# ZeayW/Multimodal-fusion-based-Pre-routing-Timing-Prediction-

Measured on AMD Instinct MI355X. Metric: train-step samples/sec, higher is better.
Workload: dtype bf16; 1 GPU; config B: 8 designs/step/GPU, 65536-node netlist, 64 levels, 256x256 tile, 1350 endpoints/design, UNet(max), bf16 operands / fp32 accumulate on the MFMA-bound contractions; U-Net activations and their gradients stored bf16, netlist tensors, statistics, parameters and gradients fp32; nodes=65536, levels=64, tile=256, endpoints_per_design=1350, cone_pruning=False, parallelism=dp1 (designs sharded, one all-reduce of the flat gradient per step), launch=one HIP graph replay per step (Adam inside)

## Files before the change

include/mmft.h:

```cpp
#ifndef MMFT_H_
#define MMFT_H_

#ifdef __cplusplus
extern "C" {
#endif

#define MMFT_OK 0
#define MMFT_ERR_BAD_ARG (-1)
#define MMFT_ERR_UNSUPPORTED (-2)
#define MMFT_ERR_LAUNCH (-3)

#define MMFT_EPI_STORE 0
#define MMFT_EPI_ACCUM 1
#define MMFT_EPI_ADD_ACT 2
#define MMFT_ACT_NONE 0
#define MMFT_ACT_RELU 1
#define MMFT_ACT_LEAKY 2
#define MMFT_POOL_MAX 0
#define MMFT_POOL_AVG 1

int mmft_version(void);
const char* mmft_last_error(void);
#define MMFT_MATH_F32 0
#define MMFT_MATH_BF16 1
// ... 232 lines not shown
int mmft_u16_pack_weights(const void* descs, int n, long long max_frag_lanes, long long* counters, int ncounters, long long inc,
                          int device, void* stream);
int mmft_u16_conv_tiles(int N, int H, int W, int* per_image);
int mmft_u16_conv3x3(const void* x, int rgb_f32, const void* wpk, void* y, float* stats, int N, int H, int W, int Ci, int Co,
                     int device, void* stream);
long long mmft_u16_conv3x3_wgrad_workspace_bytes(int N, int H, int W, int Ci, int Co);
int mmft_u16_conv3x3_wgrad_slabs(int N, int H, int W, int Ci, int Co);
int mmft_u16_conv3x3_wgrad(const void* x, int rgb_f32, const void* dy, float* dw, int accumulate, int N, int H, int W, int Ci,
                           int Co, float* workspace, long long workspace_bytes, int device, void* stream);
int mmft_u16_bn_finalize(const float* stats, int tiles_per_image, int N, int C, long long pixels_per_image, float eps,
                         const float* gamma, const float* beta, float* bnp, int device, void* stream);
int mmft_u16_bn_apply(const void* z, const float* bnp, void* a, int lda, void* pooled, int N, int H, int W, int C, int pool_mode,
                      float momentum, float* running_mean, float* running_var, int device, void* stream);
long long mmft_u16_bn_bwd_workspace_bytes(int N, long long pixels_per_image, int C);
int mmft_u16_bn_bwd(const void* g, const void* z, const float* bnp, void* dz, float* dgamma, float* dbeta, int accumulate, int N,
                    long long pixels_per_image, int C, float* workspace, long long workspace_bytes, int device, void* stream);
int mmft_u16_pool_bwd(const void* a, int lda, const void* gskip, int ldg, const void* gp, void* g, int N, int H, int W, int C,
                      int pool_mode, int device, void* stream);
int mmft_u16_convt_fwd(const void* x, const void* wpk, const float* bias, void* u, int ldu, int N, int h, int w, int Ci, int device,
                       void* stream);
int mmft_u16_convt_dgrad(const void* g, int ldu, const void* wpk_t, void* dx, int N, int h, int w, int Ci, int device, void* stream);
long long mmft_u16_convt_wgrad_workspace_bytes(int N, int h, int w, int Ci);
int mmft_u16_convt_wgrad_slabs(int N, int h, int w);
int mmft_u16_convt_wgrad(const void* x, const void* g, int ldu, float* dw, float* db, int accumulate, int N, int h, int w, int Ci,
                         float* workspace, long long workspace_bytes, int device, void* stream);
int mmft_u16_outconv_fwd(const void* x, const float* w, const float* bias, float* out, int N, int H, int W, int mode, int device,
                         void* stream);
long long mmft_u16_outconv_bwd_workspace_bytes(int N, int H, int W);
int mmft_u16_outconv_bwd_slabs(int N, int H, int W);
int mmft_u16_outconv_bwd(const void* x, const float* w, const float* bias, const float* gout, void* dx, float* dw, float* db,
                         int accumulate, int N, int H, int W, int mode, float* workspace, long long workspace_bytes, int device,
                         void* stream);

#ifdef __cplusplus
}
#endif
#endif
```

multimodal-fusion-based-pre-routing-timing-prediction-_amd/mmft/fusion.py:

```python
import numpy as np
import torch
from . import lib, ops, gradsink


def _csc_from_csr(indptr, cols, P):
    indptr = np.asarray(indptr, dtype=np.int64)
    cols = np.asarray(cols, dtype=np.int64)
    rows = np.repeat(np.arange(indptr.shape[0] - 1, dtype=np.int64), np.diff(indptr))
    order = np.argsort(cols, kind='stable')
    cptr = np.zeros(P + 1, dtype=np.int64)
    np.cumsum(np.bincount(cols, minlength=P), out=cptr[1:])
    return cptr, rows[order]


RUN_BLOCK = 64
USE_RUNS = True


def _runs_from_csr(indptr, cols, S):
    n = cols.shape[0]
    rows = indptr.shape[0] - 1
    if n == 0:
        return np.zeros(rows + 1, dtype=np.int64), np.zeros(0, dtype=np.int64), np.zeros(0, dtype=np.int64)
    new = np.ones(n, dtype=bool)
# ... 323 lines not shown

def is_unit_grad(g):
    return any(g.data_ptr() == t.data_ptr() for t in _UNIT.values())


class MseGatherFn(torch.autograd.Function):

    @staticmethod
    def forward(ctx, pred, table, idx):
        p = pred if pred.is_contiguous() else pred.contiguous()
        ops._chk(p, 'pred'); ops._chk(table, 'table')
        if p.dim() != 1 or idx.dtype != torch.int32 or idx.numel() != p.numel() or not idx.is_contiguous() or table.dim() > 2 or \
                (table.dim() == 2 and table.shape[1] != 1):
            raise ValueError('mse_gather: pred (T,), table (N,) or (N, 1), idx int32 (T,)')
        loss = torch.empty(1, dtype=torch.float32, device=p.device)
        grad = torch.empty_like(p)
        dev, st = lib.stream_args(p)
        lib.call('mmft_mse_gather_fwd_bwd', p, table, table.stride(0), idx, p.numel(), loss, grad, dev, st)
        ctx.save_for_backward(grad)
        return loss.reshape(())

    @staticmethod
    def backward(ctx, gl):
        (grad,) = ctx.saved_tensors
        return (grad if is_unit_grad(gl) else grad * gl), None, None


def mse_loss(pred, target):
    return MseFn.apply(pred, target)


def mse_loss_gather(pred, table, idx):
    return MseGatherFn.apply(pred, table, idx)


class CrossEntropyFn(torch.autograd.Function):

    @staticmethod
    def forward(ctx, logits, labels):
        z = logits if logits.is_contiguous() else logits.contiguous()
        ops._chk(z, 'logits')
        ops._chk(labels, 'labels', torch.int64)
        if z.dim() != 2 or labels.dim() != 1 or labels.numel() != z.shape[0] or not labels.is_contiguous():
            raise ValueError('cross_entropy: logits [T, C] and int64 labels [T] required')
        loss = torch.empty(1, dtype=torch.float32, device=z.device)
        grad = torch.empty_like(z)
        dev, st = lib.stream_args(z)
        lib.call('mmft_cross_entropy_fwd_bwd', z, labels, z.shape[0], z.shape[1], loss, grad, None, dev, st)
        ctx.save_for_backward(grad)
        return loss.reshape(())

    @staticmethod
    def backward(ctx, gl):
        (grad,) = ctx.saved_tensors
        return grad * gl, None


def cross_entropy_loss(logits, labels):
    return CrossEntropyFn.apply(logits, labels)


def cls_eval_sums(logits, labels):
    z = logits if logits.is_contiguous() else logits.contiguous()
    ops._chk(z, 'logits'); ops._chk(labels, 'labels', torch.int64)
    out = torch.empty(6, dtype=torch.float64, device=z.device)
    dev, st = lib.stream_args(z)
# ... 94 lines not shown
```

multimodal-fusion-based-pre-routing-timing-prediction-_amd/mmft/train.py:

```python
import os

import numpy as np
import torch
from torch import nn

from .pingraph import PinGraph
from .fusion import PathMasks, MaskedPathMap, FlatAdam, mse_loss, mse_loss_gather, cross_entropy_loss, batch_links, unit_grad


def build_models(map_size=128, out_dim=128, cell_feat_dim=36, net_feat_dim=2, cnn_outdim=128, pooling='max',
                 nlabels=1, device='cuda', seed=9294, unet=True):
    import model as M
    import Unet as U
    torch.manual_seed(seed)
    gnn = M.PathConv(out_feat_dim=out_dim, hidden_feat_dim=out_dim, cell_feat_dim=cell_feat_dim,
                     net_feat_dim=net_feat_dim, flag_attn=False, num_heads=1)
    cnn = U.UNet(pooling) if unet else M.LayoutNet(pooling)
    fcn = nn.Linear(map_size * map_size, cnn_outdim)
    nn.init.xavier_uniform_(fcn.weight, gain=nn.init.calculate_gain('relu'))
    mlp_dim = out_dim + cnn_outdim + 32
    mlp = M.MLP(mlp_dim, mlp_dim * 2, nlabels)
    pmodel = M.PathModel(gnn, None, fcn, None, None, mlp)
    return pmodel.to(device), cnn.to(device)


def trainable_parameters(pmodel, cnn):
    return [p for _, ps in parameter_buckets(pmodel, cnn) for p in ps]


def parameter_buckets(pmodel, cnn):
    skip = ('gnn.fc_net_drive.', 'gnn.fc_attn2.')
    named = [(n, p) for n, p in pmodel.named_parameters() if not n.startswith(skip)]
    head = [p for n, p in named if not n.startswith(('gnn.', 'cnn.'))]
    rest = [p for n, p in named if n.startswith(('gnn.', 'cnn.'))]
    if cnn is not None:
        seen = {id(p) for p in rest}
        rest += [p for p in cnn.parameters() if id(p) not in seen]
    return [('head', head), ('gnn+cnn', rest)]


# ... 145 lines not shown
        if cnn is not None:
            cnn.train()
        self.h = torch.zeros((self.batch.N, self.batch.out_dim), dtype=torch.float32, device=self.device)

    def forward(self, path_ids_per_design, _sel=None):
        b, g = self.batch, self.batch.graph
        ends_d, paths_d, foff_d, counts, ends_h, lv_d = _sel if _sel is not None else b.select(path_ids_per_design)
        if self.mode != 'sweep':
            self.h.zero_()
        g.ndata['h'] = self.h
        if self.mode == 'sweep':
            from . import sweep as _sweep
            cur = torch.cuda.current_stream(self.device)
            h_gnn = None
            if self.pmodel.gnn is not None:
                if self.overlap:
                    self.side.wait_stream(cur)
                    with torch.cuda.stream(self.side):
                        h_gnn = _sweep.sweep_forward_all(self.pmodel.gnn, g, b.level_nodes, ends_d,
                                                         target_order=b.end_order, cone=self.cone)
                else:
                    h_gnn = _sweep.sweep_forward_all(self.pmodel.gnn, g, b.level_nodes, ends_d, target_order=b.end_order,
                                                     cone=self.cone)
            feat = self.cnn(b.images).reshape(b.B, -1) if self.cnn is not None else None
            pm = MaskedPathMap(b.masks, paths_d, feat, foff_d if b.B > 1 else None, *b.links) \
                if feat is not None else None
            if h_gnn is not None and self.overlap and not _JOIN_LATE:
                cur.wait_stream(self.side)
                h_gnn.record_stream(cur)
            h_cnn = self.pmodel._fcn(pm) if (pm is not None and self.pmodel.fcn is not None) else None
            if h_gnn is not None and self.overlap and _JOIN_LATE:
                cur.wait_stream(self.side)
                h_gnn.record_stream(cur)
            return self.pmodel.fuse_heads(h_gnn, pm, lv_d, b.L, h_cnn=h_cnn), ends_d, ends_h
        feat = self.cnn(b.images).reshape(b.B, -1) if self.cnn is not None else None
        g.targets_unique = b.ends_unique
        hats, pos = [], 0
        for level_id in range(b.L):
            k = int(counts[level_id])
            targets = ends_d[pos:pos + k]
            path_map = None
            if k and feat is not None and self.dense_path_map:
                rows = paths_d[pos:pos + k].long()
                path_mask = torch.index_select(self._sparse_masks(), 0, rows).to_dense()
                path_map = path_mask * (feat[foff_d[pos:pos + k].long() // b.P] if b.B > 1 else feat)
            elif k and feat is not None:
                path_map = MaskedPathMap(b.masks, paths_d[pos:pos + k], feat, foff_d[pos:pos + k] if b.B > 1 else None)
                path_map.batch_links, path_map.batch_rows = b.links, (pos, paths_d.numel())
            cur = self.pmodel(g, b.level_nodes[level_id], None, targets, level_id, b.level_th[level_id], path_map)
            pos += k
            if cur is not None:
                hats.append(cur)
        return torch.cat(hats, 0), ends_d, ends_h

    def _sparse_masks(self):
        if self._sp_masks is None:
            m = self.batch.masks
            ip, cols = torch.from_numpy(m.host_indptr), torch.from_numpy(m.host_cols)
            rows = torch.repeat_interleave(torch.arange(m.num_paths), ip[1:] - ip[:-1])
            self._sp_masks = torch.sparse_coo_tensor(torch.stack([rows, cols]), torch.ones(cols.numel(), dtype=torch.int64),
                                                     (m.num_paths, m.P)).coalesce().to(self.device)
        return self._sp_masks

    def loss(self, hats, ends_d):
        if self.task == 'cls':
            labels = self.batch.graph.ndata['label'][ends_d.long()].squeeze(-1).contiguous()
            return cross_entropy_loss(hats, labels)
        return mse_loss_gather(hats, self.batch.arrival, ends_d)

    def step(self, path_ids_per_design):
        hats, ends_d, ends_h = self.forward(path_ids_per_design)
        self.last_ends = ends_d
        loss = self.loss(hats, ends_d)
        self.optim.zero_grad()
        if self.reducer is not None:
            self.reducer.begin(early=(self.mode == 'sweep'))
            loss.backward(unit_grad(self.device))
            self.reducer.finish()
        elif self.world_size > 1:
            from .dist import allreduce_sum_
            loss.backward()
            grads = [p.grad for p in self.optim.param_groups[0]['params'] if p.grad is not None]
            for g in grads:
                allreduce_sum_(g, self.world_size)
                g.mul_(1.0 / self.world_size)
            self.optim.step()
        else:
            loss.backward(unit_grad(self.device))
            self.optim.step()
        return loss.detach(), hats.detach(), ends_h.tolist()


class GraphedTrainStep:

    def __init__(self, ts, example_path_ids, warmup=3, pieces=None):
        if not ts.fused or ts.mode != 'sweep':
            raise ValueError('GraphedTrainStep needs mode="sweep" and the fused optimizer')
        self.ts = ts
        b = ts.batch
        if pieces is None:
# ... 32 lines not shown
            with torch.cuda.graph(self.graph, capture_error_mode='thread_local'):
                hats, ends_d, _ = ts.forward(None, _sel=sel)
                loss = ts.loss(hats, ends_d)
                ts.optim.zero_grad()
                loss.backward(unit_grad(ts.device))
                if ts.reducer is None:
                    ts.optim.step_captured()
                self.loss, self.hats = loss.detach(), hats.detach()
        torch.cuda.synchronize()

    def _capture_pieces(self, sel):
        from . import sweep as _sweep
        ts, b = self.ts, self.ts.batch
        pm_, cnn, g = ts.pmodel, ts.cnn, ts.batch.graph
        ends_d, paths_d, foff_d, counts, ends_h, lv_d = sel
        skip = ('gnn.fc_net_drive.', 'gnn.fc_attn2.')
        named = [(n, p) for n, p in pm_.named_parameters() if not n.startswith(skip)]
        head_params = [p for n, p in named if not n.startswith(('gnn.', 'cnn.'))]
        gnn_params = [p for n, p in named if n.startswith('gnn.')]
        cnn_params = list(cnn.parameters())
        pool = torch.cuda.graph_pool_handle()
        mk = lambda: torch.cuda.CUDAGraph()
        self.gA, self.gB, self.gH, self.gbA, self.gbB = mk(), mk(), mk(), mk(), mk()
        kw = dict(pool=pool, capture_error_mode='thread_local')
        g.ndata['h'] = ts.h
        with torch.cuda.graph(self.gA, stream=ts.side, **kw):
            h_out = _sweep.sweep_forward_all(pm_.gnn, g, b.level_nodes, ends_d, target_order=b.end_order, cone=ts.cone)
            h_leaf = h_out.detach().requires_grad_(True)
        with torch.cuda.graph(self.gB, **kw):
            feat_out = cnn(b.images).reshape(b.B, -1)
            feat_leaf = feat_out.detach().requires_grad_(True)
        with torch.cuda.graph(self.gH, **kw):
            pmap = MaskedPathMap(b.masks, paths_d, feat_leaf, foff_d if b.B > 1 else None, *b.links)
            hats = pm_.fuse_heads(h_leaf, pmap, lv_d, b.L, h_cnn=pm_._fcn(pmap))
            loss = ts.loss(hats, ends_d)
            ts.optim.zero_grad()
            torch.autograd.backward(loss, inputs=head_params + [h_leaf, feat_leaf])
            self.loss, self.hats = loss.detach(), hats.detach()
        with torch.cuda.graph(self.gbA, stream=ts.side, **kw):
            torch.autograd.backward(h_out, grad_tensors=h_leaf.grad, inputs=gnn_params)
        with torch.cuda.graph(self.gbB, **kw):
            torch.autograd.backward(feat_out, grad_tensors=feat_leaf.grad, inputs=cnn_params)
        self._keep = (h_out, h_leaf, feat_out, feat_leaf, pmap)
        self._ev = [torch.cuda.Event() for _ in range(6)]

    def step(self, path_ids_per_design):
        ts, b = self.ts, self.ts.batch
        sel = b.select(path_ids_per_design, static=self.static_idx)
        ts.last_ends = sel[0]
        if not self.pieces:
            self.graph.replay()
            if ts.reducer is not None:
                ts.reducer.after_replay()
            else:
                ts.optim.note_replay()
            return self.loss, self.hats, sel[4].tolist()
        main, side = torch.cuda.current_stream(ts.device), ts.side
        e0, eA, eH, ebA = self._ev[:4]
        e0.record(main)
        side.wait_event(e0)
        with torch.cuda.stream(side):
            self.gA.replay()
            eA.record(side)
        self.gB.replay()
        main.wait_event(eA)
        self.gH.replay()
        eH.record(main)
# ... 45 lines not shown
```

multimodal-fusion-based-pre-routing-timing-prediction-_amd/model.py:

```python
import torch as th
from torch import nn

from mmft import functional as MF
from mmft import sweep as _sweep
from mmft import cnn as _cnn
from mmft import ops as _ops
from mmft.fusion import MaskedPathMap, masked_fc, HeadLevelCtx

__all__ = ['MLP', 'PathConv', 'LayoutNet', 'PathModel', 'MaskedPathMap', 'th', 'nn']


class MLP(th.nn.Module):

    def __init__(self, *sizes, batchnorm=False, dropout=False, negative_slope=0):
        super().__init__()
        if batchnorm or dropout:
            raise NotImplementedError('MLP(batchnorm/dropout=True) is never used on the reference hot path '
                                      '(src/model.py:48-52,267; src/train.py:77) and has no HIP kernel')
        if negative_slope < 0:
            raise NotImplementedError('negative LeakyReLU slopes are not supported')
        self.negative_slope = negative_slope
        fcs = []
        for i in range(1, len(sizes)):
            fcs.append(th.nn.Linear(sizes[i - 1], sizes[i]))
            if i < len(sizes) - 1:
                fcs.append(th.nn.LeakyReLU(negative_slope=negative_slope))
        self.layers = th.nn.Sequential(*fcs)

    def forward(self, x):
        mods = list(self.layers)
        i = 0
        while i < len(mods):
            lin = mods[i]
            fused_act = i + 1 < len(mods) and isinstance(mods[i + 1], th.nn.LeakyReLU)
            x = MF.linear_act(x, lin.weight, lin.bias, self.negative_slope if fused_act else None)
            i += 2 if fused_act else 1
        return x


class PathConv(nn.Module):
# ... 206 lines not shown
            return self._fuse_level(h_gnn, self._fcn(path_map), target_list, level_id_th)
        if self.fcn is not None and len(target_list) != 0:
            h_cnn = self._fcn(path_map)
        else:
            h_cnn = None
        h_gnn = self.gnn(graph, nodes, eids, target_list, level_id) if self.gnn is not None else None
        if len(target_list) == 0:
            return None
        return self._fuse_level(h_gnn, h_cnn, target_list, level_id_th)

    def _fuse_level(self, h_gnn, h_cnn, target_list, level_id_th):
        h_global = self.mlp_alpha(level_id_th).expand(len(target_list), 32)
        if h_cnn is None:
            h = th.cat([h_gnn, h_global], dim=1)
        elif h_gnn is None:
            h = th.cat([h_cnn, h_global], dim=1)
        else:
            h = th.cat((h_gnn, h_cnn, h_global), 1)
        return self.mlp_fuse(h).squeeze(-1)

    def _lazy_ok(self, graph, target_list, path_map):
        return (LAZY_HEAD and th.is_grad_enabled() and self.gnn is not None and isinstance(self.fcn, nn.Linear)
                and isinstance(path_map, MaskedPathMap) and len(target_list) != 0 and path_map.feat_map.requires_grad)

    def forward_sweep(self, graph, level_nodes, targets, target_levels, path_map):
        T = len(targets)
        if T == 0:
            if self.gnn is not None:
                _sweep.sweep_forward_all(self.gnn, graph, level_nodes, targets)
            return None
        h_gnn = _sweep.sweep_forward_all(self.gnn, graph, level_nodes, targets) if self.gnn is not None else None
        return self.fuse_heads(h_gnn, path_map, target_levels, len(level_nodes), levels_ascending=False)

    def fuse_heads(self, h_gnn, path_map, target_levels, num_levels, h_cnn=None, levels_ascending=True):
        if h_cnn is None:
            h_cnn = self._fcn(path_map) if (self.fcn is not None and path_map is not None) else None
        cache = self.__dict__.setdefault('_level_ids', {})
        key = (num_levels, str(target_levels.device))
        lv = cache.get(key)
        if lv is None:
            lv = cache[key] = th.arange(num_levels, dtype=th.float32, device=target_levels.device).unsqueeze(1)
        h_global = MF.gather_rows(self.mlp_alpha(lv), target_levels, ascending=levels_ascending)
        parts = [p for p in (h_gnn, h_cnn, h_global) if p is not None]
        return self.mlp_fuse(MF.concat_cols(*parts) if len(parts) > 1 else parts[0]).squeeze(-1)
```

Baseline: 2448 designs/s.

## Fuse the prediction head MLP, level embedding, concat and MSE loss into HIP kernels

Adds a fused forward kernel that evaluates the level-embedding MLP, gathers and concatenates the GNN, CNN and level features in LDS, and runs the 288→576 bf16 MFMA layer with ReLU and the output dot product. It can also compute the MSE residual and per-tile loss partials in the same kernel. Matching backward, weight-gradient (split-K slabs) and final-reduction kernels replace the generic head autograd path. The goal is to remove many small launches and the intermediate tensors of the head, at the cost of hard-coded dimensions and bf16 rounding of the head operands.

```diff
diff --git a/include/mmft.h b/include/mmft.h
--- a/include/mmft.h
+++ b/include/mmft.h
@@ -288,6 +288,22 @@
                          int accumulate, int N, int H, int W, int mode, float* workspace, long long workspace_bytes, int device,
                          void* stream);
 
+int mmft_fused_head_rows(int T);
+int mmft_fused_head_partial_width(int L);
+long long mmft_fused_head_slab_floats(void);
+int mmft_fused_head_fwd(const float* h_gnn, int ld_gnn, const float* h_cnn, int ld_cnn, const int* level, int T, int L,
+                        const float* wa1, const float* ba1, const float* wa2, const float* ba2, const float* w1, const float* b1,
+                        const float* w2, const float* b2, float* pred, void* xT, void* hs, void* w1t, int Tp,
+                        const float* table, long long ld_table, const int* idx, float* dpred, double* loss_part, int device,
+                        void* stream);
+int mmft_fused_head_loss(const double* loss_part, int ntiles, int T, float* loss, int device, void* stream);
+int mmft_fused_head_bwd(const float* dpred, const void* hs, const float* w2, const void* w1t, const int* level, int T, int L, int Tp,
+                        float* dx, void* dhT, float* part, int device, void* stream);
+int mmft_fused_head_wgrad(const void* dhT, const void* xT, int Tp, const float* part, int ntiles, int L, float* slabs, float* db1,
+                          float* dw2, float* db2, float* dalpha, int device, void* stream);
+int mmft_fused_head_final(const float* slabs, float* dw1, const float* dalpha, int L, const float* wa1, const float* ba1,
+                          const float* wa2, float* dwa1, float* dba1, float* dwa2, float* dba2, int device, void* stream);
+
 #ifdef __cplusplus
 }
 #endif
diff --git a/multimodal-fusion-based-pre-routing-timing-prediction-_amd/csrc/fused_head.hip b/multimodal-fusion-based-pre-routing-timing-prediction-_amd/csrc/fused_head.hip
--- /dev/null
+++ b/multimodal-fusion-based-pre-routing-timing-prediction-_amd/csrc/fused_head.hip
@@ -0,0 +1,485 @@
+#include "common.h"
+#include "gemm_bf16.h"
+
+namespace mmft {
+namespace {
+
+constexpr int FH_DG = 128, FH_DC = 128, FH_DA = 32, FH_D = FH_DG + FH_DC + FH_DA, FH_H = 576, FH_AH = 64, FH_LMAX = 128;
+constexpr int FH_RB = 4, FH_R = 16 * FH_RB;
+constexpr int FH_XS = FH_D + 8, FH_HS = FH_H + 8;
+constexpr int FH_P0 = 2 * FH_H + 4;
+constexpr int FH_S = 8;
+constexpr int FH_WH = 64, FH_WN = 96;
+constexpr int FH_WT = (FH_H / FH_WH) * (FH_D / FH_WN);
+constexpr int FH_W1N = FH_H * FH_D;
+
+__device__ __forceinline__ float rbf(float v) { return __uint_as_float(pack_bf16(v, 0.f) << 16); }
+__device__ __forceinline__ float bf2f(unsigned short u) { return __uint_as_float((unsigned)u << 16); }
+__device__ __forceinline__ float relu1(float v) { return v > 0.f ? v : 0.f; }
+__device__ __forceinline__ bf16x8 cvt8(f32x4 a, f32x4 b) {
+  u32x4 u = {pack_bf16(a.x, a.y), pack_bf16(a.z, a.w), pack_bf16(b.x, b.y), pack_bf16(b.z, b.w)};
+  return __builtin_bit_cast(bf16x8, u);
+}
+__device__ __forceinline__ void col8_store(unsigned short* dst, const unsigned short* src, int stride) {
+  u32x4 u;
+  u.x = (unsigned)src[0] | ((unsigned)src[stride] << 16);
+  u.y = (unsigned)src[2 * stride] | ((unsigned)src[3 * stride] << 16);
+  u.z = (unsigned)src[4 * stride] | ((unsigned)src[5 * stride] << 16);
+  u.w = (unsigned)src[6 * stride] | ((unsigned)src[7 * stride] << 16);
+  *reinterpret_cast<u32x4*>(dst) = u;
+}
+
+__global__ void __launch_bounds__(256) MMFT_NO_PACKED_F32 fused_head_fwd_kernel(
+    const float* __restrict__ hg, int ldg, const float* __restrict__ hc, int ldc, const int* __restrict__ level, int T, int L,
+    const float* __restrict__ wa1, const float* __restrict__ ba1, const float* __restrict__ wa2, const float* __restrict__ ba2,
+    const float* __restrict__ w1, const float* __restrict__ b1, const float* __restrict__ w2, const float* __restrict__ b2,
+    float* __restrict__ pred, unsigned short* __restrict__ xT, unsigned short* __restrict__ hs, unsigned short* __restrict__ w1t, int Tp,
+    const float* __restrict__ table, long long ldt, const int* __restrict__ idx, float* __restrict__ dpred, double* __restrict__ lpart) {
+  __shared__ __attribute__((aligned(16))) unsigned short xs[FH_R * FH_XS];
+  __shared__ float sal[FH_LMAX * FH_DA];
+  __shared__ float red[4][FH_R];
+  __shared__ double dred[FH_R];
+  __shared__ int slv[FH_R];
+  const int tid = threadIdx.x, lane = tid & 63, wave = tid >> 6, r16 = lane & 15, q = lane >> 4;
+  const int t0 = blockIdx.x * FH_R, nrows = min(FH_R, T - t0);
+
+  float* sw = reinterpret_cast<float*>(xs);
+  float *swa1 = sw, *sba1 = sw + FH_AH, *sba2 = sw + 2 * FH_AH, *swa2 = sw + 2 * FH_AH + FH_DA;
+  if (tid < FH_AH) { swa1[tid] = rbf(wa1[tid]); sba1[tid] = ba1[tid]; }
+  if (tid < FH_DA) sba2[tid] = ba2[tid];
+  for (int e = tid; e < FH_DA * FH_AH; e += 256) swa2[(e >> 6) * 65 + (e & 63)] = rbf(wa2[e]);
+  if (tid < FH_R) slv[tid] = tid < nrows ? level[t0 + tid] : -1;
+  __syncthreads();
+  for (int e = tid; e < L * 4; e += 256) {
+    const int l = e >> 2, c0 = (e & 3) * 8;
+    const float lf = rbf((float)l);
+    float acc[8] = {0.f, 0.f, 0.f, 0.f, 0.f, 0.f, 0.f, 0.f};
+    for (int j = 0; j < FH_AH; ++j) {
+      const float hr = rbf(relu1(fmaf(lf, swa1[j], sba1[j])));
+#pragma unroll
+      for (int c = 0; c < 8; ++c) acc[c] = fmaf(hr, swa2[(c0 + c) * 65 + j], acc[c]);
+    }
+#pragma unroll
+    for (int c = 0; c < 8; ++c) sal[l * FH_DA + c0 + c] = acc[c] + sba2[c0 + c];
+  }
+  __syncthreads();
+
+  for (int g = tid; g < FH_R * (FH_D / 8); g += 256) {
+    const int r = g / (FH_D / 8), col = (g % (FH_D / 8)) * 8;
+    f32x4 a = {0.f, 0.f, 0.f, 0.f}, b = a;
+    if (r < nrows) {
+      const long long t = t0 + r;
+      const float* p = nullptr;
+      if (col < FH_DG) p = hg + t * ldg + col;
+      else if (col < FH_DG + FH_DC) p = hc + t * ldc + (col - FH_DG);
+      else if (slv[r] >= 0 && slv[r] < L) p = sal + slv[r] * FH_DA + (col - FH_DG - FH_DC);
+      if (p) { a = *reinterpret_cast<const f32x4*>(p); b = *reinterpret_cast<const f32x4*>(p + 4); }
+    }
+    *reinterpret_cast<bf16x8*>(xs + r * FH_XS + col) = cvt8(a, b);
+  }
+  __syncthreads();
+  if (xT)
+    for (int g = tid; g < FH_D * (FH_R / 8); g += 256) {
+      const int r8 = g % (FH_R / 8), n = g / (FH_R / 8);
+      col8_store(xT + (long long)n * Tp + t0 + r8 * 8, xs + r8 * 8 * FH_XS + n, FH_XS);
+    }
+  if (w1t)
+    for (int g = blockIdx.x * 256 + tid; g < FH_D * (FH_H / 8); g += gridDim.x * 256) {
+      const int n = g % FH_D, h0 = (g / FH_D) * 8;
+      const float* p = w1 + (long long)h0 * FH_D + n;
+      const f32x4 a = {p[0], p[FH_D], p[2 * FH_D], p[3 * FH_D]}, b = {p[4 * FH_D], p[5 * FH_D], p[6 * FH_D], p[7 * FH_D]};
+      *reinterpret_cast<bf16x8*>(w1t + (long long)n * FH_H + h0) = cvt8(a, b);
+    }
+
+  f32x4 acc[FH_RB][9];
+#pragma unroll
+  for (int i = 0; i < FH_RB; ++i)
+#pragma unroll
+    for (int j = 0; j < 9; ++j) acc[i][j] = f32x4{0.f, 0.f, 0.f, 0.f};
+  const float* wrow = w1 + (long long)(wave * 144 + r16) * FH_D + q * 8;
+#pragma unroll 1
+  for (int ks = 0; ks < FH_D / 32; ++ks) {
+    bf16x8 af[9];
+#pragma unroll
+    for (int j = 0; j < 9; ++j) {
+      const float* p = wrow + (long long)j * 16 * FH_D + ks * 32;
+      af[j] = cvt8(*reinterpret_cast<const f32x4*>(p), *reinterpret_cast<const f32x4*>(p + 4));
+    }
+#pragma unroll
+    for (int i = 0; i < FH_RB; ++i) {
+      const bf16x8 xf = *reinterpret_cast<const bf16x8*>(xs + (i * 16 + r16) * FH_XS + ks * 32 + q * 8);
+#pragma unroll
+      for (int j = 0; j < 9; ++j) acc[i][j] = __builtin_amdgcn_mfma_f32_16x16x32_bf16(af[j], xf, acc[i][j], 0, 0, 0);
+    }
+  }
+  float s[FH_RB];
+#pragma unroll
+  for (int i = 0; i < FH_RB; ++i) s[i] = 0.f;
+#pragma unroll
+  for (int j = 0; j < 9; ++j) {
+    const int hc0 = wave * 144 + j * 16 + q * 4;
+    const f32x4 bb = *reinterpret_cast<const f32x4*>(b1 + hc0);
+    const f32x4 ww = *reinterpret_cast<const f32x4*>(w2 + hc0);
+    const float w2r[4] = {rbf(ww.x), rbf(ww.y), rbf(ww.z), rbf(ww.w)};
+#pragma unroll
+    for (int i = 0; i < FH_RB; ++i) {
+      const f32x4 v = acc[i][j];
+      const unsigned lo = pack_bf16(relu1(v.x + bb.x), relu1(v.y + bb.y)), hi = pack_bf16(relu1(v.z + bb.z), relu1(v.w + bb.w));
+      const int row = i * 16 + r16;
+      if (row < nrows)
+        *reinterpret_cast<unsigned long long*>(hs + (long long)(t0 + row) * FH_H + hc0) = ((unsigned long long)hi << 32) | lo;
+      s[i] = fmaf(__uint_as_float(lo << 16), w2r[0], s[i]);
+      s[i] = fmaf(__uint_as_float(lo & 0xffff0000u), w2r[1], s[i]);
+      s[i] = fmaf(__uint_as_float(hi << 16), w2r[2], s[i]);
+      s[i] = fmaf(__uint_as_float(hi & 0xffff0000u), w2r[3], s[i]);
+    }
+  }
+#pragma unroll
+  for (int i = 0; i < FH_RB; ++i) {
+    float v = s[i];
+    v += __shfl_xor(v, 16);
+    v += __shfl_xor(v, 32);
+    if (q == 0) red[wave][i * 16 + r16] = v;
+  }
+  __syncthreads();
+  if (tid < FH_R) {
+    double dd = 0.0;
+    if (tid < nrows) {
+      const int t = t0 + tid;
+      const float p = ((red[0][tid] + red[1][tid]) + red[2][tid]) + red[3][tid] + b2[0];
+      pred[t] = p;
+      if (dpred) {
+        const float d = p - table[(long long)idx[t] * ldt];
+        dpred[t] = d * (2.0f / (float)T);
+        dd = (double)d * (double)d;
+      }
+    }
+    dred[tid] = dd;
+  }
+  if (lpart) {
+    __syncthreads();
+    if (tid == 0) {
+      double a = 0.0;
+      for (int r = 0; r < FH_R; ++r) a += dred[r];
+      lpart[blockIdx.x] = a;
+    }
+  }
+}
+
+__global__ void __launch_bounds__(256) fused_head_loss_kernel(const double* __restrict__ part, int n, int T, float* __restrict__ loss) {
+  __shared__ double red[256];
+  double s = 0.0;
+  for (int i = threadIdx.x; i < n; i += 256) s += part[i];
+  red[threadIdx.x] = s;
+  __syncthreads();
+  for (int o = 128; o > 0; o >>= 1) {
+    if ((int)threadIdx.x < o) red[threadIdx.x] += red[threadIdx.x + o];
+    __syncthreads();
+  }
+  if (threadIdx.x == 0) loss[0] = (float)(red[0] / (double)T);
+}
+
+inline int bwd_lds_bytes(int L) { return FH_R * FH_HS * 2 + L * FH_DA * 4 + FH_R * 33 * 4 + FH_R * 8; }
+
+__global__ void __launch_bounds__(256) MMFT_NO_PACKED_F32 fused_head_bwd_kernel(
+    const float* __restrict__ gp, const unsigned short* __restrict__ hs, const float* __restrict__ w2,
+    const unsigned short* __restrict__ w1t, const int* __restrict__ level, int T, int L, int Tp, float* __restrict__ dx,
+    unsigned short* __restrict__ dhT, float* __restrict__ part, int pw) {
+  extern __shared__ __attribute__((aligned(16))) unsigned char fh_lds[];
+  unsigned short* dhs = reinterpret_cast<unsigned short*>(fh_lds);
+  float* tab = reinterpret_cast<float*>(fh_lds + FH_R * FH_HS * 2);
+  float* sdA = tab + L * FH_DA;
+  float* sg = sdA + FH_R * 33;
+  int* slv = reinterpret_cast<int*>(sg + FH_R);
+  const int tid = threadIdx.x, lane = tid & 63, wave = tid >> 6, r16 = lane & 15, q = lane >> 4;
+  const int t0 = blockIdx.x * FH_R, nrows = min(FH_R, T - t0);
+  float* prt = part + (long long)blockIdx.x * pw;
+
+  for (int e = tid; e < L * FH_DA; e += 256) tab[e] = 0.f;
+  if (tid < FH_R) {
+    sg[tid] = tid < nrows ? gp[t0 + tid] : 0.f;
+    slv[tid] = tid < nrows ? level[t0 + tid] : -1;
+  }
+  __syncthreads();
+  for (int c = tid; c < FH_H; c += 256) {
+    const float w2r = rbf(w2[c]);
+    float sdb = 0.f, sdw = 0.f;
+    for (int r = 0; r < FH_R; ++r) {
+      unsigned short out = 0;
+      if (r < nrows) {
+        const unsigned short hb = hs[(long long)(t0 + r) * FH_H + c];
+        const float gr = rbf(sg[r]);
+        const float dh = hb ? gr * w2r : 0.f;
+        sdb += dh;
+        sdw = fmaf(gr, bf2f(hb), sdw);
+        out = (unsigned short)(pack_bf16(dh, 0.f) & 0xffffu);
+      }
+      dhs[r * FH_HS + c] = out;
+    }
+    prt[c] = sdb;
+    prt[FH_H + c] = sdw;
+  }
+  if (tid == 0) {
+    float a = 0.f;
+    for (int r = 0; r < nrows; ++r) a += sg[r];
+    prt[2 * FH_H] = a;
+    prt[2 * FH_H + 1] = prt[2 * FH_H + 2] = prt[2 * FH_H + 3] = 0.f;
+  }
+  __syncthreads();
+  for (int g = tid; g < FH_H * (FH_R / 8); g += 256) {
+    const int r8 = g % (FH_R / 8), h = g / (FH_R / 8);
+    col8_store(dhT + (long long)h * Tp + t0 + r8 * 8, dhs + r8 * 8 * FH_HS + h, FH_HS);
+  }
+  f32x4 acc[FH_RB][5];
+#pragma unroll
+  for (int i = 0; i < FH_RB; ++i)
+#pragma unroll
+    for (int m = 0; m < 5; ++m) acc[i][m] = f32x4{0.f, 0.f, 0.f, 0.f};
+#pragma unroll 1
+  for (int ks = 0; ks < FH_H / 32; ++ks) {
+    bf16x8 bfr[FH_RB];
+#pragma unroll
+    for (int i = 0; i < FH_RB; ++i) bfr[i] = *reinterpret_cast<const bf16x8*>(dhs + (i * 16 + r16) * FH_HS + ks * 32 + q * 8);
+#pragma unroll
+    for (int m = 0; m < 5; ++m) {
+      const int cb = wave + 4 * m;
+      if (cb >= FH_D / 16) continue;
+      const bf16x8 af = *reinterpret_cast<const bf16x8*>(w1t + (long long)(cb * 16 + r16) * FH_H + ks * 32 + q * 8);
+#pragma unroll
+      for (int i = 0; i < FH_RB; ++i) acc[i][m] = __builtin_amdgcn_mfma_f32_16x16x32_bf16(af, bfr[i], acc[i][m], 0, 0, 0);
+    }
+  }
+#pragma unroll
+  for (int m = 0; m < 5; ++m) {
+    const int cb = wave + 4 * m;
+    if (cb >= FH_D / 16) continue;
+    const int n = cb * 16 + q * 4;
+#pragma unroll
+    for (int i = 0; i < FH_RB; ++i) {
+      const int row = i * 16 + r16;
+      if (row < nrows) *reinterpret_cast<f32x4*>(dx + (long long)(t0 + row) * FH_D + n) = acc[i][m];
+      if (n >= FH_DG + FH_DC) {
+        float* d = sdA + row * 33 + (n - FH_DG - FH_DC);
+        d[0] = acc[i][m].x; d[1] = acc[i][m].y; d[2] = acc[i][m].z; d[3] = acc[i][m].w;
+      }
+    }
+  }
+  __syncthreads();
+  if (tid < FH_DA) {
+    int cur = -1;
+    float a = 0.f;
+    for (int r = 0; r < nrows; ++r) {
+      const int lv = slv[r];
+      if (lv != cur) {
+        if (cur >= 0 && cur < L) tab[cur * FH_DA + tid] += a;
+        cur = lv;
+        a = 0.f;
+      }
+      a += sdA[r * 33 + tid];
+    }
+    if (cur >= 0 && cur < L) tab[cur * FH_DA + tid] += a;
+  }
+  __syncthreads();
+  for (int e = tid; e < L * FH_DA; e += 256) prt[FH_P0 + e] = tab[e];
+}
+
+__global__ void __launch_bounds__(256) MMFT_NO_PACKED_F32 fused_head_wgrad_kernel(
+    const unsigned short* __restrict__ dhT, const unsigned short* __restrict__ xT, int Tp, float* __restrict__ slabs,
+    const float* __restrict__ part, int ntiles, int pw, float* __restrict__ db1, float* __restrict__ dw2, float* __restrict__ db2,
+    float* __restrict__ dalpha) {
+  const int tid = threadIdx.x;
+  if ((int)blockIdx.x >= FH_WT * FH_S) {
+    __shared__ float sred[8][32];
+    const int cl = tid & 31, g = tid >> 5, col = ((int)blockIdx.x - FH_WT * FH_S) * 32 + cl;
+    float a = 0.f;
+    if (col < pw)
+      for (int t = g; t < ntiles; t += 8) a += part[(long long)t * pw + col];
+    sred[g][cl] = a;
+    __syncthreads();
+    if (tid < 32 && col < pw) {
+      float v = sred[0][cl];
+#pragma unroll
+      for (int k = 1; k < 8; ++k) v += sred[k][cl];
+      if (col < FH_H) db1[col] = v;
+      else if (col < 2 * FH_H) dw2[col - FH_H] = v;
+      else if (col == 2 * FH_H) db2[0] = v;
+      else if (col >= FH_P0) dalpha[col - FH_P0] = v;
+    }
+    return;
+  }
+  const int lane = tid & 63, wave = tid >> 6, r16 = lane & 15, q = lane >> 4;
+  const int tile = blockIdx.x % FH_WT, s = blockIdx.x / FH_WT;
+  const int h0 = (tile % (FH_H / FH_WH)) * FH_WH + (wave & 1) * 32, n0 = (tile / (FH_H / FH_WH)) * FH_WN + (wave >> 1) * 48;
+  const int kc = ((Tp + FH_S - 1) / FH_S + 31) / 32 * 32;
+  const int tb = s * kc, te = min(Tp, tb + kc);
+  f32x4 acc[2][3];
+#pragma unroll
+  for (int a = 0; a < 2; ++a)
+#pragma unroll
+    for (int b = 0; b < 3; ++b) acc[a][b] = f32x4{0.f, 0.f, 0.f, 0.f};
+  const unsigned short* hp = dhT + (long long)(h0 + r16) * Tp + q * 8;
+  const unsigned short* xp = xT + (long long)(n0 + r16) * Tp + q * 8;
+  for (int t = tb; t < te; t += 32) {
+    bf16x8 hf[2], xf[3];
+#pragma unroll
+    for (int a = 0; a < 2; ++a) hf[a] = *reinterpret_cast<const bf16x8*>(hp + (long long)a * 16 * Tp + t);
+#pragma unroll
+    for (int b = 0; b < 3; ++b) xf[b] = *reinterpret_cast<const bf16x8*>(xp + (long long)b * 16 * Tp + t);
+#pragma unroll
+    for (int a = 0; a < 2; ++a)
+#pragma unroll
+      for (int b = 0; b < 3; ++b) acc[a][b] = __builtin_amdgcn_mfma_f32_16x16x32_bf16(xf[b], hf[a], acc[a][b], 0, 0, 0);
+  }
+  float* out = slabs + (long long)s * FH_W1N;
+#pragma unroll
+  for (int a = 0; a < 2; ++a)
+#pragma unroll
+    for (int b = 0; b < 3; ++b)
+      *reinterpret_cast<f32x4*>(out + (long long)(h0 + a * 16 + r16) * FH_D + n0 + b * 16 + q * 4) = acc[a][b];
+}
+
+constexpr int FH_FIN_BLOCKS = FH_W1N / 4 / 256;
+
+__global__ void __launch_bounds__(256) MMFT_NO_PACKED_F32 fused_head_final_kernel(
+    const float* __restrict__ slabs, float* __restrict__ dw1, const float* __restrict__ dalpha, int L,
+    const float* __restrict__ wa1, const float* __restrict__ ba1, const float* __restrict__ wa2,
+    float* __restrict__ dwa1, float* __restrict__ dba1, float* __restrict__ dwa2, float* __restrict__ dba2) {
+  const int tid = threadIdx.x;
+  if ((int)blockIdx.x < FH_FIN_BLOCKS) {
+    const long long e = ((long long)blockIdx.x * 256 + tid) * 4;
+    f32x4 v = *reinterpret_cast<const f32x4*>(slabs + e);
+#pragma unroll
+    for (int s = 1; s < FH_S; ++s) v += *reinterpret_cast<const f32x4*>(slabs + (long long)s * FH_W1N + e);
+    *reinterpret_cast<f32x4*>(dw1 + e) = v;
+    return;
+  }
+  __shared__ float sda[FH_LMAX * FH_DA];
+  __shared__ float sdh[FH_LMAX * FH_AH];
+  __shared__ float swa1[FH_AH], sba1[FH_AH], swa2[FH_DA * 65];
+  for (int e = tid; e < L * FH_DA; e += 256) sda[e] = dalpha[e];
+  if (tid < FH_AH) { swa1[tid] = rbf(wa1[tid]); sba1[tid] = ba1[tid]; }
+  for (int e = tid; e < FH_DA * FH_AH; e += 256) swa2[(e >> 6) * 65 + (e & 63)] = rbf(wa2[e]);
+  __syncthreads();
+  if (tid < FH_DA) {
+    float a = 0.f;
+    for (int l = 0; l < L; ++l) a += sda[l * FH_DA + tid];
+    dba2[tid] = a;
+  }
+  for (int e = tid; e < FH_DA * FH_AH; e += 256) {
+    const int c = e >> 6, j = e & 63;
+    float a = 0.f;
+    for (int l = 0; l < L; ++l) a = fmaf(rbf(sda[l * FH_DA + c]), rbf(relu1(fmaf(rbf((float)l), swa1[j], sba1[j]))), a);
+    dwa2[e] = a;
+  }
+  for (int e = tid; e < L * FH_AH; e += 256) {
+    const int l = e >> 6, j = e & 63;
+    float a = 0.f;
+    if (fmaf(rbf((float)l), swa1[j], sba1[j]) > 0.f)
+      for (int c = 0; c < FH_DA; ++c) a = fmaf(rbf(sda[l * FH_DA + c]), swa2[c * 65 + j], a);
+    sdh[e] = a;
+  }
+  __syncthreads();
+  if (tid < FH_AH) {
+    float a = 0.f, b = 0.f;
+    for (int l = 0; l < L; ++l) {
+      const float d = sdh[l * FH_AH + tid];
+      a = fmaf(rbf(d), rbf((float)l), a);
+      b += d;
+    }
+    dwa1[tid] = a;
+    dba1[tid] = b;
+  }
+}
+
+DynLdsOnce g_bwd_lds;
+
+}
+}
+
+using namespace mmft;
+
+extern "C" {
+
+int mmft_fused_head_rows(int T) { return T > 0 ? cdiv(T, FH_R) * FH_R : 0; }
+
+int mmft_fused_head_partial_width(int L) { return FH_P0 + L * FH_DA; }
+
+int mmft_fused_head_fwd(const float* h_gnn, int ld_gnn, const float* h_cnn, int ld_cnn, const int* level, int T, int L,
+                        const float* wa1, const float* ba1, const float* wa2, const float* ba2, const float* w1, const float* b1,
+                        const float* w2, const float* b2, float* pred, void* xT, void* hs, void* w1t, int Tp,
+                        const float* table, long long ld_table, const int* idx, float* dpred, double* loss_part, int device,
+                        void* stream) {
+  MMFT_REQUIRE(h_gnn && h_cnn && level && wa1 && ba1 && wa2 && ba2 && w1 && b1 && w2 && b2 && pred && hs, "fused_head_fwd: null pointer");
+  MMFT_REQUIRE(T > 0 && T <= (1 << 24) && L >= 1 && L <= FH_LMAX && Tp == mmft_fused_head_rows(T), "fused_head_fwd: bad sizes");
+  MMFT_REQUIRE(aligned16(h_gnn) && aligned16(h_cnn) && ld_gnn % 4 == 0 && ld_cnn % 4 == 0 && ld_gnn >= FH_DG && ld_cnn >= FH_DC &&
+                   aligned16(w1) && aligned16(b1) && aligned16(w2) && aligned16(xT) && aligned16(hs) && aligned16(w1t),
+               "fused_head_fwd: rows must be 16-byte aligned");
+  MMFT_REQUIRE(!dpred || (table && idx && loss_part && ld_table >= 1), "fused_head_fwd: loss needs table, idx and partials");
+  DeviceGuard dg(device);
+  hipStream_t st = (hipStream_t)stream;
+  const int nt = Tp / FH_R;
+  const double flops = 2.0 * Tp * FH_D * FH_H + 2.0 * Tp * FH_H + 2.0 * nt * L * FH_AH * FH_DA;
+  const double bytes = (double)T * (FH_DG + FH_DC) * 4 + T * 8.0 + FH_W1N * 4.0 + (xT ? Tp * FH_D * 2.0 : 0.0) +
+                       T * FH_H * 2.0 + T * 4.0 + (w1t ? FH_W1N * 2.0 : 0.0) + (dpred ? T * 12.0 + nt * 8.0 : 0.0);
+  MMFT_LAUNCH("fused_head_fwd_kernel", flops, bytes, fused_head_fwd_kernel, dim3(nt), dim3(256), st, h_gnn, ld_gnn, h_cnn, ld_cnn,
+              level, T, L, wa1, ba1, wa2, ba2, w1, b1, w2, b2, pred, (unsigned short*)xT, (unsigned short*)hs,
+              (unsigned short*)w1t, Tp, table, ld_table, idx, dpred, loss_part);
+  return check_launch("fused_head_fwd");
+}
+
+int mmft_fused_head_loss(const double* loss_part, int ntiles, int T, float* loss, int device, void* stream) {
+  MMFT_REQUIRE(loss_part && loss && ntiles > 0 && T > 0, "fused_head_loss: bad args");
+  DeviceGuard dg(device);
+  MMFT_LAUNCH("fused_head_loss_kernel", (double)ntiles, ntiles * 8.0 + 4.0, fused_head_loss_kernel, dim3(1), dim3(256),
+              (hipStream_t)stream, loss_part, ntiles, T, loss);
+  return check_launch("fused_head_loss");
+}
+
+int mmft_fused_head_bwd(const float* dpred, const void* hs, const float* w2, const void* w1t, const int* level, int T, int L, int Tp,
+                        float* dx, void* dhT, float* part, int device, void* stream) {
+  MMFT_REQUIRE(dpred && hs && w2 && w1t && level && dx && dhT && part, "fused_head_bwd: null pointer");
+  MMFT_REQUIRE(T > 0 && T <= (1 << 24) && L >= 1 && L <= FH_LMAX && Tp == mmft_fused_head_rows(T), "fused_head_bwd: bad sizes");
+  MMFT_REQUIRE(aligned16(dx) && aligned16(dhT) && aligned16(w1t) && aligned16(part), "fused_head_bwd: unaligned buffer");
+  DeviceGuard dg(device);
+  const int lds = bwd_lds_bytes(L);
+  int rc = ensure_dyn_lds(g_bwd_lds, (const void*)fused_head_bwd_kernel, bwd_lds_bytes(FH_LMAX), "fused_head_bwd");
+  if (rc != MMFT_OK) return rc;
+  const int nt = Tp / FH_R, pw = FH_P0 + L * FH_DA;
+  const double flops = 2.0 * Tp * FH_H * FH_D + 4.0 * Tp * FH_H;
+  const double bytes = T * 8.0 + T * FH_H * 2.0 + FH_W1N * 2.0 + T * FH_D * 4.0 + Tp * FH_H * 2.0 + nt * (double)pw * 4;
+  MMFT_LAUNCH_LDS("fused_head_bwd_kernel", flops, bytes, fused_head_bwd_kernel, dim3(nt), dim3(256), lds, (hipStream_t)stream,
+                  dpred, (const unsigned short*)hs, w2, (const unsigned short*)w1t, level, T, L, Tp, dx, (unsigned short*)dhT, part,
+                  pw);
+  return check_launch("fused_head_bwd");
+}
+
+long long mmft_fused_head_slab_floats(void) { return (long long)FH_S * FH_W1N; }
+
+int mmft_fused_head_wgrad(const void* dhT, const void* xT, int Tp, const float* part, int ntiles, int L, float* slabs, float* db1,
+                          float* dw2, float* db2, float* dalpha, int device, void* stream) {
+  MMFT_REQUIRE(dhT && xT && part && slabs && db1 && dw2 && db2 && dalpha, "fused_head_wgrad: null pointer");
+  MMFT_REQUIRE(Tp > 0 && Tp % FH_R == 0 && ntiles == Tp / FH_R && L >= 1 && L <= FH_LMAX, "fused_head_wgrad: bad sizes");
+  MMFT_REQUIRE(aligned16(dhT) && aligned16(xT) && aligned16(slabs), "fused_head_wgrad: unaligned buffer");
+  DeviceGuard dg(device);
+  const int pw = FH_P0 + L * FH_DA, nred = cdiv(pw, 32);
+  const double flops = 2.0 * Tp * FH_H * FH_D + (double)ntiles * pw;
+  const double bytes = Tp * (FH_H + FH_D) * 2.0 + FH_S * (double)FH_W1N * 4 + (double)ntiles * pw * 4 + pw * 4.0;
+  MMFT_LAUNCH("fused_head_wgrad_kernel", flops, bytes, fused_head_wgrad_kernel, dim3(FH_WT * FH_S + nred), dim3(256),
+              (hipStream_t)stream, (const unsigned short*)dhT, (const unsigned short*)xT, Tp, slabs, part, ntiles, pw, db1, dw2, db2,
+              dalpha);
+  return check_launch("fused_head_wgrad");
+}
+
+int mmft_fused_head_final(const float* slabs, float* dw1, const float* dalpha, int L, const float* wa1, const float* ba1,
+                          const float* wa2, float* dwa1, float* dba1, float* dwa2, float* dba2, int device, void* stream) {
+  MMFT_REQUIRE(slabs && dw1 && dalpha && wa1 && ba1 && wa2 && dwa1 && dba1 && dwa2 && dba2, "fused_head_final: null pointer");
+  MMFT_REQUIRE(L >= 1 && L <= FH_LMAX && aligned16(slabs) && aligned16(dw1), "fused_head_final: bad args");
+  DeviceGuard dg(device);
+  const double flops = (double)FH_S * FH_W1N + 2.0 * L * FH_AH * FH_DA * 2;
+  const double bytes = (FH_S + 1.0) * FH_W1N * 4 + L * FH_DA * 4.0 + (FH_AH * 2 + FH_DA * FH_AH) * 8.0;
+  MMFT_LAUNCH("fused_head_final_kernel", flops, bytes, fused_head_final_kernel, dim3(FH_FIN_BLOCKS + 1), dim3(256),
+              (hipStream_t)stream, slabs, dw1, dalpha, L, wa1, ba1, wa2, dwa1, dba1, dwa2, dba2);
+  return check_launch("fused_head_final");
+}
+
+}
diff --git a/multimodal-fusion-based-pre-routing-timing-prediction-_amd/mmft/fusion.py b/multimodal-fusion-based-pre-routing-timing-prediction-_amd/mmft/fusion.py
--- a/multimodal-fusion-based-pre-routing-timing-prediction-_amd/mmft/fusion.py
+++ b/multimodal-fusion-based-pre-routing-timing-prediction-_amd/mmft/fusion.py
@@ -379,6 +379,133 @@
 
 def mse_loss_gather(pred, table, idx):
     return MseGatherFn.apply(pred, table, idx)
+
+
+import os as _os
+
+FUSED_HEAD = _os.environ.get('MMFT_FUSED_HEAD', '0') == '1'
+
+
+def _relu_mlp(m, sizes):
+    mods = list(getattr(m, 'layers', ()))
+    if len(mods) != 3 or getattr(m, 'negative_slope', None) != 0 or not isinstance(mods[1], torch.nn.LeakyReLU):
+        return None
+    l1, l2 = mods[0], mods[2]
+    if not (isinstance(l1, torch.nn.Linear) and isinstance(l2, torch.nn.Linear)) or l1.bias is None or l2.bias is None:
+        return None
+    if (l1.in_features, l1.out_features, l2.out_features) != tuple(sizes):
+        return None
+    ps = (l1.weight, l1.bias, l2.weight, l2.bias)
+    if any(p.dtype != torch.float32 or not p.is_contiguous() or p.data_ptr() % 16 for p in ps):
+        return None
+    return ps
+
+
+def fused_head_params(mlp_alpha, mlp_fuse, h_gnn, h_cnn, num_levels):
+    if not FUSED_HEAD or h_gnn is None or h_cnn is None or not 1 <= num_levels <= 128:
+        return None
+    for h, w in ((h_gnn, 128), (h_cnn, 128)):
+        if h.dim() != 2 or h.dtype != torch.float32 or h.shape[1] != w or h.stride(1) != 1 or h.stride(0) % 4 or \
+                h.data_ptr() % 16 or h.device.type != 'cuda':
+            return None
+    if h_gnn.shape[0] != h_cnn.shape[0] or h_gnn.shape[0] == 0 or lib.get_math_mode() != 'bf16':
+        return None
+    pa, pf = _relu_mlp(mlp_alpha, (1, 64, 32)), _relu_mlp(mlp_fuse, (288, 576, 1))
+    return pa + pf if pa is not None and pf is not None else None
+
+
+class FusedHeadFn(torch.autograd.Function):
+
+    @staticmethod
+    def forward(ctx, h_gnn, h_cnn, level, num_levels, loss_target, wa1, ba1, wa2, ba2, w1, b1, w2, b2):
+        T, L, dev = h_gnn.shape[0], int(num_levels), h_gnn.device
+        if level.dtype != torch.int32 or level.numel() != T or not level.is_contiguous():
+            raise ValueError('fused head: int32 level ids, one per row')
+        Tp = lib.query('mmft_fused_head_rows', T)
+        nt = Tp // 64
+        pred = torch.empty(T, dtype=torch.float32, device=dev)
+        xT = torch.empty(288 * Tp, dtype=torch.int16, device=dev)
+        hs = torch.empty(Tp * 576, dtype=torch.int16, device=dev)
+        w1t = torch.empty(288 * 576, dtype=torch.int16, device=dev)
+        table = idx = dpred = lpart = None
+        ld = 1
+        if loss_target is not None:
+            table, idx = loss_target
+            if table.dim() > 2 or (table.dim() == 2 and table.shape[1] != 1) or idx.dtype != torch.int32 or \
+                    idx.numel() != T or not idx.is_contiguous():
+                raise ValueError('fused head loss: table (N,) or (N, 1), idx int32 (T,)')
+            ops._chk(table, 'table')
+            ld = table.stride(0)
+            dpred = torch.empty(T, dtype=torch.float32, device=dev)
+            lpart = torch.empty(nt, dtype=torch.float64, device=dev)
+        devi, st = lib.stream_args(h_gnn)
+        lib.call('mmft_fused_head_fwd', h_gnn, h_gnn.stride(0), h_cnn, h_cnn.stride(0), level, T, L, wa1, ba1, wa2, ba2, w1, b1,
+                 w2, b2, pred, xT, hs, w1t, Tp, table, ld, idx, dpred, lpart, devi, st)
+        ctx.T, ctx.L, ctx.Tp = T, L, Tp
+        ctx.keep = (level, xT, hs, w1t, wa1, ba1, wa2, w2)
+        ctx.sinks = [gradsink.of(p) for p in (w1, b1, w2, b2, wa1, ba1, wa2, ba2)]
+        ctx.shapes = [p.shape for p in (w1, b1, w2, b2, wa1, ba1, wa2, ba2)]
+        ctx.fused_mse = (dpred, lpart, idx) if dpred is not None else None
+        return pred
+
+    @staticmethod
+    def backward(ctx, gpred):
+        T, L, Tp = ctx.T, ctx.L, ctx.Tp
+        level, xT, hs, w1t, wa1, ba1, wa2, w2 = ctx.keep
+        g = gpred if (gpred.dtype == torch.float32 and gpred.is_contiguous()) else gpred.float().contiguous()
+        dev = g.device
+        devi, st = lib.stream_args(g)
+        nt = Tp // 64
+        pw = lib.query('mmft_fused_head_partial_width', L)
+        dx = torch.empty((T, 288), dtype=torch.float32, device=dev)
+        dhT = torch.empty(576 * Tp, dtype=torch.int16, device=dev)
+        part = torch.empty(nt * pw, dtype=torch.float32, device=dev)
+        lib.call('mmft_fused_head_bwd', g, hs, w2, w1t, level, T, L, Tp, dx, dhT, part, devi, st)
+
+        def _grads(*outs):
+            outs = [o if o is not None else torch.empty(s, dtype=torch.float32, device=dev) for o, s in zip(outs, ctx.shapes)]
+            dw1, db1, dw2, db2, dwa1, dba1, dwa2, dba2 = outs
+            slabs = torch.empty(lib.query('mmft_fused_head_slab_floats'), dtype=torch.float32, device=dev)
+            dalpha = torch.empty(L * 32, dtype=torch.float32, device=dev)
+            lib.call('mmft_fused_head_wgrad', dhT, xT, Tp, part, nt, L, slabs, db1, dw2, db2, dalpha, devi, st)
+            lib.call('mmft_fused_head_final', slabs, dw1, dalpha, L, wa1, ba1, wa2, dwa1, dba1, dwa2, dba2, devi, st)
+            return outs
+        grads = gradsink.deliver_many(ctx.sinks, _grads)
+        grads = [None if gr is None else gr.reshape(s) for gr, s in zip(grads, ctx.shapes)]
+        gw1, gb1, gw2, gb2, gwa1, gba1, gwa2, gba2 = grads
+        out = [dx[:, :128], dx[:, 128:256], None, None, None, gwa1, gba1, gwa2, gba2, gw1, gb1, gw2, gb2]
+        return tuple(o if need else None for o, need in zip(out, ctx.needs_input_grad))
+
+
+class FusedMseFn(torch.autograd.Function):
+
+    @staticmethod
+    def forward(ctx, pred, dpred, lpart):
+        loss = torch.empty(1, dtype=torch.float32, device=pred.device)
+        lib.call('mmft_fused_head_loss', lpart, lpart.numel(), pred.numel(), loss, *lib.stream_args(pred))
+        ctx.dpred = dpred
+        return loss.reshape(())
+
+    @staticmethod
+    def backward(ctx, gl):
+        return (ctx.dpred if is_unit_grad(gl) else ctx.dpred * gl), None, None
+
+
+def fused_head(h_gnn, h_cnn, level, num_levels, params, loss_target=None):
+    pred = FusedHeadFn.apply(h_gnn, h_cnn, level, num_levels, loss_target, *params)
+    if loss_target is not None:
+        pred._mmft_fused_mse = (pred.grad_fn, loss_target[1])
+    return pred
+
+
+def fused_mse_loss(pred, idx):
+    tag = getattr(pred, '_mmft_fused_mse', None)
+    if tag is None or tag[1] is not idx or pred.grad_fn is not tag[0]:
+        return None
+    dpred, lpart, _ = tag[0].fused_mse if hasattr(tag[0], 'fused_mse') else (None, None, None)
+    if dpred is None:
+        return None
+    return FusedMseFn.apply(pred, dpred, lpart)
 
 
 class CrossEntropyFn(torch.autograd.Function):
diff --git a/multimodal-fusion-based-pre-routing-timing-prediction-_amd/mmft/train.py b/multimodal-fusion-based-pre-routing-timing-prediction-_amd/mmft/train.py
--- a/multimodal-fusion-based-pre-routing-timing-prediction-_amd/mmft/train.py
+++ b/multimodal-fusion-based-pre-routing-timing-prediction-_amd/mmft/train.py
@@ -5,7 +5,8 @@
 from torch import nn
 
 from .pingraph import PinGraph
-from .fusion import PathMasks, MaskedPathMap, FlatAdam, mse_loss, mse_loss_gather, cross_entropy_loss, batch_links, unit_grad
+from .fusion import PathMasks, MaskedPathMap, FlatAdam, mse_loss, mse_loss_gather, cross_entropy_loss, batch_links, unit_grad, \
+    fused_mse_loss
 
 
 def build_models(map_size=128, out_dim=128, cell_feat_dim=36, net_feat_dim=2, cnn_outdim=128, pooling='max',
@@ -217,7 +218,7 @@
             if h_gnn is not None and self.overlap and _JOIN_LATE:
                 cur.wait_stream(self.side)
                 h_gnn.record_stream(cur)
-            return self.pmodel.fuse_heads(h_gnn, pm, lv_d, b.L, h_cnn=h_cnn), ends_d, ends_h
+            return self.pmodel.fuse_heads(h_gnn, pm, lv_d, b.L, h_cnn=h_cnn, loss_target=self._loss_target(ends_d)), ends_d, ends_h
         feat = self.cnn(b.images).reshape(b.B, -1) if self.cnn is not None else None
         g.targets_unique = b.ends_unique
         hats, pos = [], 0
@@ -247,10 +248,16 @@
                                                      (m.num_paths, m.P)).coalesce().to(self.device)
         return self._sp_masks
 
+    def _loss_target(self, ends_d):
+        return (self.batch.arrival, ends_d) if self.task == 'reg' else None
+
     def loss(self, hats, ends_d):
         if self.task == 'cls':
             labels = self.batch.graph.ndata['label'][ends_d.long()].squeeze(-1).contiguous()
             return cross_entropy_loss(hats, labels)
+        fused = fused_mse_loss(hats, ends_d)
+        if fused is not None:
+            return fused
         return mse_loss_gather(hats, self.batch.arrival, ends_d)
 
     def step(self, path_ids_per_design):
@@ -349,7 +356,7 @@
             feat_leaf = feat_out.detach().requires_grad_(True)
         with torch.cuda.graph(self.gH, **kw):
             pmap = MaskedPathMap(b.masks, paths_d, feat_leaf, foff_d if b.B > 1 else None, *b.links)
-            hats = pm_.fuse_heads(h_leaf, pmap, lv_d, b.L, h_cnn=pm_._fcn(pmap))
+            hats = pm_.fuse_heads(h_leaf, pmap, lv_d, b.L, h_cnn=pm_._fcn(pmap), loss_target=ts._loss_target(ends_d))
             loss = ts.loss(hats, ends_d)
             ts.optim.zero_grad()
             torch.autograd.backward(loss, inputs=head_params + [h_leaf, feat_leaf])
diff --git a/multimodal-fusion-based-pre-routing-timing-prediction-_amd/model.py b/multimodal-fusion-based-pre-routing-timing-prediction-_amd/model.py
--- a/multimodal-fusion-based-pre-routing-timing-prediction-_amd/model.py
+++ b/multimodal-fusion-based-pre-routing-timing-prediction-_amd/model.py
@@ -5,7 +5,7 @@
 from mmft import sweep as _sweep
 from mmft import cnn as _cnn
 from mmft import ops as _ops
-from mmft.fusion import MaskedPathMap, masked_fc, HeadLevelCtx
+from mmft.fusion import MaskedPathMap, masked_fc, HeadLevelCtx, fused_head, fused_head_params
 
 __all__ = ['MLP', 'PathConv', 'LayoutNet', 'PathModel', 'MaskedPathMap', 'th', 'nn']
 
@@ -278,9 +278,13 @@
         h_gnn = _sweep.sweep_forward_all(self.gnn, graph, level_nodes, targets) if self.gnn is not None else None
         return self.fuse_heads(h_gnn, path_map, target_levels, len(level_nodes), levels_ascending=False)
 
-    def fuse_heads(self, h_gnn, path_map, target_levels, num_levels, h_cnn=None, levels_ascending=True):
+    def fuse_heads(self, h_gnn, path_map, target_levels, num_levels, h_cnn=None, levels_ascending=True, loss_target=None):
         if h_cnn is None:
             h_cnn = self._fcn(path_map) if (self.fcn is not None and path_map is not None) else None
+        params = fused_head_params(self.mlp_alpha, self.mlp_fuse, h_gnn, h_cnn, num_levels)
+        if params is not None:
+            lv32 = target_levels if target_levels.dtype == th.int32 else target_levels.to(th.int32)
+            return fused_head(h_gnn, h_cnn, lv32.contiguous(), num_levels, params, loss_target)
         cache = self.__dict__.setdefault('_level_ids', {})
         key = (num_levels, str(target_levels.device))
         lv = cache.get(key)
```

Result: no change. 2444 designs/s (median of 2 runs) (-0.1%).
